# mankeyboy/ASR-FeatExt-OpenCL

Measured on NVIDIA B200. Metric: mfcc_delta_delta2_frames_per_s, higher is better.
Workload: dtype f32

## Files before the change

### asr-featext-opencl_b200/csrc/afe_fused.cuh

```cuda
#pragma once
#include <cfloat>

#include "afe_fft.cuh"
#include "afe_mel.cuh"

namespace afe {

struct Tile {
    long long pcm_off;
    long long out_row0;
    int T;
    int t0;
    int nout;
    int group;
    int tile0;
    int ntiles;
    int flags;
    int pad_;
};
constexpr int kTileNoStats = 1;
constexpr int kTileQ1All = 2;

constexpr int kMaxBanks = 64;
constexpr int kMaxWl4 = (2 * 257 + 10 * kMaxBanks + 3) / 4;
constexpr int kMagStride = 260;
__host__ __device__ constexpr int mag_row(int f) { return 8 * (f >> 3) + ((f >> 1) & 3) + 4 * (f & 1); }

struct MelConst {
    float4 wl4[kMaxWl4];
    float4 dct4[kMaxBanks][4];
    int desc[kMaxBanks];
    short wstart[8];
    int mma_unit[8][2];
    int mma_boff[8][2];
};

struct FusedArgs {
    const int16_t *pcm;
    float *out;
    const Tile *tiles;
    const float2 *window2, *tw_a, *tw_p;
    double *partials;
    int *counters;
    int cluster_norm;
    int tile_base;
    int norm_type, norm_after_dyn;
#ifdef AFE_DEVTOOLS
    int debug_skip;
#endif
    int W, S, nb, dct_len, cols, width, l1, l2, nstreams;
    int q1;
    int use_tma;
    int stats_rows_mode;
    int stats_count;
    int use_last;
    float *g_mean, *g_scale;
    int *work_counter;
    unsigned *flags;
    unsigned epoch;
    int ntiles_launch;
    float pre;
    int blk_ntiles, blk_T, blk_t_first, blk_n_out, blk_nout, blk_spec, blk_spec_q1;
    const float4 *mma_bfrag, *mma_dfrag;
    int stats_kind;
    int tc_max;
    float rden1, rden2;
};

constexpr int kRoundFrames = 32;
constexpr int kMaxFusedThreads = 256;

struct FusedSmem {
    int off_mbar, off_mags, off_part, off_warp, warp_bytes, w_pcm, w_scratch, pcm_bytes, off_dhat, off_dd, off_red,
        off_cep, total;
};

inline int align_up(int v, int a) { return (v + a - 1) / a * a; }

template <int N2>
FusedSmem fused_smem_layout(int kFusedWarps, int S, int cols, int tc_max, int nout_max, int l2, int nstreams)
{
    using C = dev::FftCfg<N2>;
    const int kWarpFrames = kRoundFrames / kFusedWarps;
    FusedSmem L;
    int o = 0;
    L.off_mbar = o; o += align_up(kFusedWarps * 8, 16);
    L.off_mags = o; o += align_up((kRoundFrames * kMagStride + 16) * 4, 16);
    L.pcm_bytes = align_up(((kWarpFrames - 1) * S + N2) * 2, 16) + 16;
    L.w_pcm = 0;
    L.warp_bytes = L.pcm_bytes;
    o = align_up(o, 128);
    L.off_warp = o; o += kFusedWarps * L.warp_bytes;
    o = align_up(o, 128);
    const int scratch = kFusedWarps * align_up(C::FPW * C::SCR * 8, 16);
    const int part = kFusedWarps * 4 * kRoundFrames * 16;
    L.w_scratch = align_up(C::FPW * C::SCR * 8, 16);
    L.off_part = o; o += scratch > part ? scratch : part;
    const int dhat = nstreams >= 2 ? align_up((nout_max + 2 * l2) * cols * 4, 16) : 0;
    const int dd = nstreams >= 3 ? align_up(nout_max * cols * 4, 16) : 0;
    L.off_dhat = L.off_mags;
    L.off_dd = L.off_dhat + dhat;
    L.off_red = L.off_dd + dd;
    const int phase3_end = L.off_red + kMaxFusedThreads * 4 * 8;
    if (phase3_end > o) o = align_up(phase3_end, 128);
    L.off_cep = o; o += align_up(tc_max * cols * 4, 16);
    L.total = o;
    return L;
}

namespace dev {

__device__ __forceinline__ uint32_t smem_u32(const void *p) { return (uint32_t)__cvta_generic_to_shared(p); }

__device__ __forceinline__ void mbar_init(uint64_t *bar, int count)
{
    asm volatile("mbarrier.init.shared::cta.b64 [%0], %1;" ::"r"(smem_u32(bar)), "r"(count));
}
__device__ __forceinline__ void mbar_expect_tx(uint64_t *bar, uint32_t bytes)
{
    asm volatile("mbarrier.arrive.expect_tx.shared::cta.b64 _, [%0], %1;" ::"r"(smem_u32(bar)), "r"(bytes) : "memory");
}
__device__ __forceinline__ void mbar_wait(uint64_t *bar, uint32_t parity)
{
    for (uint32_t spin = 0; spin < (1u << 24); spin++) {
        uint32_t done;
        asm volatile(
            "{\n\t.reg .pred p;\n\t"
            "mbarrier.try_wait.parity.shared::cta.b64 p, [%1], %2;\n\t"
            "selp.u32 %0, 1, 0, p;\n\t}"
            : "=r"(done)
            : "r"(smem_u32(bar)), "r"(parity)
            : "memory");
        if (done) return;
    }
    __trap();
}
__device__ __forceinline__ void tma_bulk_g2s(void *dst, const void *src, uint32_t bytes, uint64_t *bar)
{
    asm volatile("cp.async.bulk.shared::cluster.global.mbarrier::complete_tx::bytes [%0], [%1], %2, [%3];" ::"r"(
                     smem_u32(dst)),
                 "l"(src), "r"(bytes), "r"(smem_u32(bar))
                 : "memory");
}

__device__ __forceinline__ float4 lds128(uint32_t addr)
{
    float4 v;
    asm volatile("ld.shared.v4.f32 {%0, %1, %2, %3}, [%4];" : "=f"(v.x), "=f"(v.y), "=f"(v.z), "=f"(v.w) : "r"(addr));
    return v;
}
__device__ __forceinline__ uint32_t opaque(uint32_t v)
{
    asm volatile("" : "+r"(v));
    return v;
}

__device__ __forceinline__ void cluster_sync()
{
    asm volatile("barrier.cluster.arrive.release.aligned;\n\tbarrier.cluster.wait.acquire.aligned;" ::: "memory");
}
__device__ __forceinline__ uint32_t cluster_size()
{
    uint32_t n;
    asm volatile("mov.u32 %0, %%cluster_nctarank;" : "=r"(n));
    return n;
}
__device__ __forceinline__ double ld_peer_f64(const double *local, uint32_t rank)
{
    uint32_t peer;
    double v;
    asm volatile("mapa.shared::cluster.u32 %0, %1, %2;" : "=r"(peer) : "r"(smem_u32(local)), "r"(rank));
    asm volatile("ld.shared::cluster.f64 %0, [%1];" : "=d"(v) : "r"(peer) : "memory");
    return v;
}

__device__ __forceinline__ int clampi(int v, int lo, int hi) { return v < lo ? lo : (v > hi ? hi : v); }

}

namespace dev {

__device__ __forceinline__ float delta_num(const float *p, int stride, int L)
{
    if (L == 3) {
        float num = p[stride] - p[-stride];
        num = fmaf(2.f, p[2 * stride] - p[-2 * stride], num);
        return fmaf(3.f, p[3 * stride] - p[-3 * stride], num);
    }
    float num = 0.f;
    for (int l = 1; l <= L; l++) num = fmaf((float)l, p[l * stride] - p[-l * stride], num);
    return num;
}

template <int KIND>
__device__ __forceinline__ void write_rows(float *__restrict__ orow, const float *__restrict__ src, int r_off, int rpp, int nout,
                                           int rq, int rs, int cols, int width, int D, double &sum, double &sumsq, float &mn,
                                           float &mx)
{
    const int ostep = rpp * width, sstep = rpp * cols;
    orow += r_off * width;
    src += r_off * cols;
    for (int r = r_off; r < nout; r += rpp, orow += ostep, src += sstep) {
        const float sval = *src;
        *orow = r >= rq ? src[-D * cols] : sval;
        if (KIND >= 1 && r < rs) {
            sum += (double)sval;
            if (KIND >= 2) sumsq += (double)__fmul_rn(sval, sval);
            if (KIND >= 3) { mn = fminf(mn, sval); mx = fmaxf(mx, sval); }
        }
    }
}

template <int MODE>
__device__ __forceinline__ void phase3_l3(const int KIND, const FusedArgs &a, const Tile &tl, const float *__restrict__ s_cep,
                                          int c0f, int c1f, double *__restrict__ s_red3, int tid, int nthreads, int rs,
                                          const float *norm3 = nullptr)
{
    constexpr int R = 8;
    const int cols = a.cols, width = a.width, T = tl.T, t0 = tl.t0, nout = tl.nout;
    const int rp = nthreads / cols, g = tid / cols, c = tid - g * cols;
    if (g >= rp) return;
    const int q1 = (tl.flags & kTileQ1All) ? 2 : a.q1;
    const int rq = q1 ? (q1 == 2 ? 0 : max(0, T - 6 - t0)) : nout;
    const float rden1 = a.rden1, rden2 = a.rden2;
    double sum[3] = {0.0, 0.0, 0.0}, sumsq[3] = {0.0, 0.0, 0.0};
    float mn[3] = {FLT_MAX, FLT_MAX, FLT_MAX}, mx[3] = {-FLT_MAX, -FLT_MAX, -FLT_MAX};
    float nm[3] = {0.f, 0.f, 0.f}, ns[3] = {1.f, 1.f, 1.f};
    if (MODE == 2) {
#pragma unroll
        for (int k = 0; k < 3; k++) { nm[k] = norm3[k]; ns[k] = norm3[3 + k]; }
    }
    const bool cmn = a.norm_type == AFE_NORM_CMN;
    float *obase = a.out + (tl.out_row0 + t0) * (long long)width + c;
    for (int r0 = g * R; r0 < (MODE == 1 ? rs : nout); r0 += rp * R) {
        float x[R + 12], dh[R + 6];
#pragma unroll
        for (int i = 0; i < R + 12; i++)
            x[i] = s_cep[(clampi(t0 + r0 - 6 + i, c0f, c1f - 1) - c0f) * cols + c];
#pragma unroll
        for (int j = 0; j < R + 6; j++) {
            float num = x[j + 4] - x[j + 2];
            num = fmaf(2.f, x[j + 5] - x[j + 1], num);
            num = fmaf(3.f, x[j + 6] - x[j], num);
            dh[j] = __fmul_rn(num, rden1);
        }
        float *orow = obase + (long long)r0 * width;
#pragma unroll
        for (int r = 0; r < R; r++, orow += width) {
            const int row = r0 + r;
            if (row >= nout) break;
            float num = dh[r + 4] - dh[r + 2];
            num = fmaf(2.f, dh[r + 5] - dh[r + 1], num);
            num = fmaf(3.f, dh[r + 6] - dh[r], num);
            const float v[3] = {x[r + 6], dh[r + 3], __fmul_rn(num, rden2)};
            if (MODE == 0) {
                orow[0] = row >= rq ? x[r] : v[0];
                orow[cols] = v[1];
                orow[2 * cols] = v[2];
            } else if (MODE == 2) {
                const float w0 = row >= rq ? x[r] : v[0];
                orow[0] = cmn ? w0 - nm[0] : (w0 - nm[0]) * ns[0];
                orow[cols] = cmn ? v[1] - nm[1] : (v[1] - nm[1]) * ns[1];
                orow[2 * cols] = cmn ? v[2] - nm[2] : (v[2] - nm[2]) * ns[2];
            }
            if (MODE != 2 && KIND >= 1 && row < rs) {
#pragma unroll
                for (int k = 0; k < 3; k++) {
                    sum[k] += (double)v[k];
                    if (KIND >= 2) sumsq[k] += (double)__fmul_rn(v[k], v[k]);
                    if (KIND >= 3) { mn[k] = fminf(mn[k], v[k]); mx[k] = fmaxf(mx[k], v[k]); }
                }
            }
        }
    }
    if (MODE != 2) {
#pragma unroll
        for (int k = 0; k < 3; k++) {
            double *p = s_red3 + ((g * width) + k * cols + c) * 4;
            p[0] = sum[k]; p[1] = sumsq[k]; p[2] = (double)mn[k]; p[3] = (double)mx[k];
        }
    }
}

}

namespace dev {
__device__ __forceinline__ void mma_tf32(float (&c)[4], const uint32_t (&a)[4], uint32_t b0, uint32_t b1)
{
    asm volatile("mma.sync.aligned.m16n8k8.row.col.f32.tf32.tf32.f32 {%0, %1, %2, %3}, {%4, %5, %6, %7}, {%8, %9}, {%0, %1, %2, %3};"
                 : "+f"(c[0]), "+f"(c[1]), "+f"(c[2]), "+f"(c[3])
                 : "r"(a[0]), "r"(a[1]), "r"(a[2]), "r"(a[3]), "r"(b0), "r"(b1));
}
__device__ __forceinline__ void mma_3xtf32(float (&c)[4], const float (&av)[4], const float4 b)
{
    uint32_t ah[4], al[4];
#pragma unroll
    for (int i = 0; i < 4; i++) {
        ah[i] = __float_as_uint(av[i]) & 0xffffe000u;
        al[i] = __float_as_uint(av[i] - __uint_as_float(ah[i]));
    }
    mma_tf32(c, al, __float_as_uint(b.x), __float_as_uint(b.y));
    mma_tf32(c, ah, __float_as_uint(b.z), __float_as_uint(b.w));
    mma_tf32(c, ah, __float_as_uint(b.x), __float_as_uint(b.y));
}
}

namespace dev {
__device__ __forceinline__ Tile load_tile(const FusedArgs &a, int idx)
{
    if (a.blk_ntiles == 0) return a.tiles[idx];
    const int D = a.l1 + a.l2;
    Tile tl;
    tl.pcm_off = 0; tl.out_row0 = -(long long)a.blk_t_first; tl.T = a.blk_T; tl.group = 0; tl.tile0 = 0;
    tl.ntiles = a.blk_ntiles + a.blk_spec; tl.pad_ = 0;
    if (idx < a.blk_ntiles) {
        tl.t0 = a.blk_t_first + idx * a.blk_nout;
        tl.nout = min(a.blk_nout, a.blk_t_first + a.blk_n_out - tl.t0);
        tl.flags = 0;
    } else {
        tl.t0 = a.blk_T - D; tl.nout = D;
        tl.flags = kTileNoStats | (a.blk_spec_q1 ? kTileQ1All : 0);
    }
    return tl;
}

constexpr int kSeqTiles = 32, kSegs = 6;
__host__ __device__ inline int seg_len(int ntiles) { return ntiles <= kSeqTiles ? ntiles : (ntiles + kSegs - 1) / kSegs; }

static __device__ unsigned g_opaque_zero = 0;

__device__ __forceinline__ void sum_records(const double *__restrict__ partials, int width, int c, int t_begin, int t_end,
                                            double &s0, double &s1, double &lo, double &hi, int tstep = 1)
{
    s0 = 0.0; s1 = 0.0; lo = (double)FLT_MAX; hi = -(double)FLT_MAX;
    constexpr int U = 8;
    const size_t stride = (size_t)width * 4 * tstep;
    const double *p = partials + ((size_t)t_begin * width + c) * 4;
    const int last = t_end - 1;
    const unsigned z = *reinterpret_cast<volatile unsigned *>(&g_opaque_zero);
    for (int t = t_begin; t < t_end; t += U * tstep, p += U * stride) {
        double2 a[U], b[U];
#pragma unroll
        for (int k = 0; k < U; k++) {
            const double2 *q = reinterpret_cast<const double2 *>(t + k * tstep <= last ? p + k * stride : p);
            a[k] = q[0];
            b[k] = q[1];
        }
        unsigned all = 0;
#pragma unroll
        for (int k = 0; k < U; k++)
            all |= (unsigned)__double2hiint(a[k].x) | (unsigned)__double2hiint(a[k].y) | (unsigned)__double2hiint(b[k].x) |
                   (unsigned)__double2hiint(b[k].y);
        a[0].x = __hiloint2double(__double2hiint(a[0].x) | (int)(all & z), __double2loint(a[0].x));
#pragma unroll
        for (int k = 0; k < U; k++) {
            const bool ok = t + k * tstep <= last;
            s0 += ok ? a[k].x : 0.0; s1 += ok ? a[k].y : 0.0;
            lo = fmin(lo, ok ? b[k].x : (double)FLT_MAX); hi = fmax(hi, ok ? b[k].y : -(double)FLT_MAX);
        }
    }
}

__device__ __forceinline__ void group_total(const double *__restrict__ partials, int width, int tile0, int ntiles, int tid,
                                            int nthreads, double *s_seg, int c_of_tid, double &s0, double &s1, double &lo, double &hi)
{
    if (ntiles <= kSeqTiles) {
        if (tid < width) sum_records(partials, width, c_of_tid, tile0, tile0 + ntiles, s0, s1, lo, hi);
        return;
    }
    const int len = seg_len(ntiles);
    for (int i = tid; i < kSegs * width; i += nthreads) {
        const int seg = i / width, c = i - seg * width;
        const int b = min(ntiles, seg * len), e = min(ntiles, b + len);
        double a0, a1, l, h;
        sum_records(partials, width, c, tile0 + b, tile0 + e, a0, a1, l, h);
        double *o = s_seg + (size_t)i * 4;
        o[0] = a0; o[1] = a1; o[2] = l; o[3] = h;
    }
    __syncthreads();
    if (tid < width) {
        s0 = 0.0; s1 = 0.0; lo = (double)FLT_MAX; hi = -(double)FLT_MAX;
        for (int seg = 0; seg < kSegs; seg++) {
            const double *o = s_seg + ((size_t)seg * width + c_of_tid) * 4;
            s0 += o[0]; s1 += o[1];
            lo = fmin(lo, o[2]); hi = fmax(hi, o[3]);
        }
    }
}

__device__ __forceinline__ void normalise_tile_rows(float *__restrict__ out, const Tile &tl, int width, int norm_type,
                                                    const float *__restrict__ mean, const float *__restrict__ scale, float *s_ms)
{
    float *base = out + (tl.out_row0 + tl.t0) * (long long)width;
    const int n = tl.nout * width;
    for (int i = threadIdx.x; i < width; i += blockDim.x) {
        s_ms[i] = __ldcg(mean + (long long)tl.group * width + i);
        s_ms[width + i] = norm_type == AFE_NORM_CMN ? 1.f : __ldcg(scale + (long long)tl.group * width + i);
    }
    __syncthreads();
    const float *m = s_ms, *sc = s_ms + width;
    const bool cmn = norm_type == AFE_NORM_CMN;
    const int head = min(n, (int)(((16 - (reinterpret_cast<uintptr_t>(base) & 15)) & 15) >> 2));
    const int n4 = (n - head) >> 2, tail0 = head + 4 * n4;
    if ((int)threadIdx.x < head) {
        const int i = threadIdx.x;
        const float v = __ldcg(base + i) - m[i % width];
        base[i] = cmn ? v : v * sc[i % width];
    }
    if ((int)threadIdx.x < n - tail0) {
        const int i = tail0 + threadIdx.x, c = i % width;
        const float v = __ldcg(base + i) - m[c];
        base[i] = cmn ? v : v * sc[c];
    }
    float4 *p4 = reinterpret_cast<float4 *>(base + head);
    int c = (head + 4 * (int)threadIdx.x) % width;
    const int cstep = (4 * (int)blockDim.x) % width;
    constexpr int U = 4;
    const int bd = blockDim.x;
    for (int j = threadIdx.x; j < n4; j += U * bd) {
        float4 v[U];
#pragma unroll
        for (int k = 0; k < U; k++)
            if (j + k * bd < n4) v[k] = __ldcg(p4 + j + k * bd);
#pragma unroll
        for (int k = 0; k < U; k++) {
            if (j + k * bd < n4) {
                int c1 = c + 1; if (c1 >= width) c1 -= width;
                int c2 = c1 + 1; if (c2 >= width) c2 -= width;
                int c3 = c2 + 1; if (c3 >= width) c3 -= width;
                float4 w = v[k];
                w.x -= m[c]; w.y -= m[c1]; w.z -= m[c2]; w.w -= m[c3];
                if (!cmn) { w.x *= sc[c]; w.y *= sc[c1]; w.z *= sc[c2]; w.w *= sc[c3]; }
                p4[j + k * bd] = w;
            }
            c += cstep; if (c >= width) c -= width;
        }
    }
}

__device__ __forceinline__ void normalise_role(const FusedArgs &a, const Tile tl, float *s_ms)
{
    if (threadIdx.x == 0) {
        unsigned v = 0;
        for (unsigned spin = 0; spin < (1u << 26); spin++) {
            asm volatile("ld.acquire.gpu.global.u32 %0, [%1];" : "=r"(v) : "l"(a.flags + tl.group) : "memory");
            if (v == a.epoch) break;
            __nanosleep(128);
        }
        if (v != a.epoch) __trap();
    }
    __syncthreads();
    normalise_tile_rows(a.out, tl, a.width, a.norm_type, a.g_mean, a.g_scale, s_ms);
}
}

template <int N2, int NZ, int kFusedWarps, int KF, bool PRE, bool MMA = false>
__global__ void __launch_bounds__(32 * kFusedWarps, 2)
k_fused_mfcc(const FusedArgs a, const FusedSmem L, const __grid_constant__ MelConst mc)
{
    constexpr bool FAST = false;
    using C = dev::FftCfg<N2>;
    constexpr int kFusedThreads = 32 * kFusedWarps, kWarpFrames = kRoundFrames / kFusedWarps;
    constexpr int R = C::R, FPW = C::FPW, SCR = C::SCR;
    static_assert(kWarpFrames % FPW == 0, "a warp's frames must fill whole FFT calls");
    extern __shared__ __align__(128) unsigned char smem[];
    float *s_mags = reinterpret_cast<float *>(smem + L.off_mags);
    float *s_cep = reinterpret_cast<float *>(smem + L.off_cep);

    const int tid = threadIdx.x, lane = tid & 31;
    const int warp = __shfl_sync(0xffffffffu, tid >> 5, 0);
    const int lf = lane % R, fw = lane / R;
    unsigned char *wbase = smem + L.off_warp + warp * L.warp_bytes;
    uint64_t *w_mbar = reinterpret_cast<uint64_t *>(smem + L.off_mbar) + warp;
    unsigned char *w_pcm = wbase + L.w_pcm;
    float2 *w_scratch = reinterpret_cast<float2 *>(smem + L.off_part + warp * L.w_scratch);

    int tile_local = blockIdx.x;
    if (a.work_counter) {
        __shared__ int s_role;
        if (tid == 0) {
            const int t = atomicAdd(a.work_counter, 1);
            if (t == (int)gridDim.x - 1) *a.work_counter = 0;
            s_role = t;
        }
        __syncthreads();
        tile_local = s_role;
        if (tile_local >= a.ntiles_launch) {
            const int n_norm = (int)gridDim.x - a.ntiles_launch;
            for (int j = tile_local - a.ntiles_launch; j < a.ntiles_launch; j += n_norm) {
                dev::normalise_role(a, dev::load_tile(a, a.tile_base + j), reinterpret_cast<float *>(smem));
                __syncthreads();
            }
            return;
        }
    }
    const int tile_idx = a.tile_base + tile_local;
    const Tile tl = dev::load_tile(a, tile_idx);
    const int q1 = (tl.flags & kTileQ1All) ? 2 : a.q1;
    const int D = a.l1 + a.l2, cols = a.cols;
    const int c0f = max(0, tl.t0 - D), c1f = min(tl.T, tl.t0 + tl.nout + D);
    const int ncomp = c1f - c0f;
    const int nrounds = (ncomp + kRoundFrames - 1) / kRoundFrames;
    const int16_t *wpcm = a.pcm + tl.pcm_off + (long long)(c0f + warp * kWarpFrames) * a.S;
    auto warp_frames = [&](int r) { return min(kWarpFrames, ncomp - r * kRoundFrames - warp * kWarpFrames); };
    auto issue_tma = [&](int r) {
        const int nf = warp_frames(r);
        if (nf <= 0) return;
        const uint32_t bytes = (uint32_t)((((nf - 1) * a.S + a.W) * 2 + 15) & ~15);
        asm volatile("fence.proxy.async.shared::cta;" ::: "memory");
        dev::mbar_expect_tx(w_mbar, bytes);
        dev::tma_bulk_g2s(w_pcm, wpcm + (long long)r * kRoundFrames * a.S, bytes, w_mbar);
    };
    if (a.use_tma && lane == 0) {
        dev::mbar_init(w_mbar, 1);
        asm volatile("fence.mbarrier_init.release.cluster;" ::: "memory");
        issue_tma(0);
    }
    dev::LaneConsts<N2, NZ> lc;
    dev::load_lane_consts<N2, NZ>(lc, a.window2, a.tw_a, a.tw_p, lf);
    for (int i = tid; i < (kRoundFrames * kMagStride + 16) / 4; i += kFusedThreads)
        reinterpret_cast<float4 *>(s_mags)[i] = make_float4(0.f, 0.f, 0.f, 0.f);
    __syncthreads();

    const uint32_t mrow_s = dev::opaque(dev::smem_u32(s_mags) + mag_row(lane) * kMagStride * 4);
    uint32_t parity = 0;
    for (int r = 0; r < nrounds; r++) {
        const int f0 = r * kRoundFrames;
        const int nfr = min(kRoundFrames, ncomp - f0);
        const int nfw = warp_frames(r);
        if (nfw > 0) {
            if (a.use_tma) {
                dev::mbar_wait(w_mbar, parity);
                parity ^= 1;
            } else {
                const int16_t *src = wpcm + (long long)f0 * a.S;
                const int n = (nfw - 1) * a.S + a.W;
                int16_t *dst = reinterpret_cast<int16_t *>(w_pcm);
                if ((reinterpret_cast<uintptr_t>(src) & 3) == 0) {
                    const uint32_t *s32 = reinterpret_cast<const uint32_t *>(src);
                    uint32_t *d32 = reinterpret_cast<uint32_t *>(dst);
                    for (int i = lane; i < n / 2; i += 32) d32[i] = __ldg(s32 + i);
                    if ((n & 1) && lane == 0) dst[n - 1] = src[n - 1];
                } else
                    for (int i = lane; i < n; i += 32) dst[i] = src[i];
                __syncwarp();
            }
#pragma unroll
            for (int it = 0; it < kWarpFrames / FPW; it++) {
                if (it * FPW >= nfw) break;
#ifdef AFE_DEVTOOLS
                if (a.debug_skip & 1) break;
#endif
                const int fl = it * FPW + fw;
                const int fr = warp * kWarpFrames + fl;
                const uint32_t *words = reinterpret_cast<const uint32_t *>(w_pcm) + ((fl * a.S) >> 1);
                dev::fft_frame_mag<N2, NZ, true, false, PRE>(words, lc, w_scratch + fw * SCR, s_mags + mag_row(fr) * kMagStride, lf, a.pre);
            }
            if (a.use_tma && lane == 0 && r + 1 < nrounds) issue_tma(r + 1);
        }
        __syncthreads();

        if constexpr (MMA) {
            const int g = lane >> 2, t = lane & 3;
#pragma unroll 1
            for (int ui = 0; ui < 2; ui++) {
                const int ud = mc.mma_unit[warp][ui];
                if (ud < 0) break;
                const int m = ud & 1, j = (ud >> 4) & 15, s0 = (ud >> 8) & 255, ns = (ud >> 16) & 255;
                const float4 *bf = a.mma_bfrag + (size_t)mc.mma_boff[warp][ui] * 32 + lane;
                const int row = 16 * m + (g >> 1) + 4 * (g & 1);
                const float *r0 = s_mags + row * kMagStride + 8 * s0 + t, *r1 = r0 + 8 * kMagStride;
                float e[4] = {0.f, 0.f, 0.f, 0.f};
#pragma unroll 2
                for (int s = 0; s < ns; s++, r0 += 8, r1 += 8, bf += 32) {
                    const float4 b = __ldg(bf);
                    const float av[4] = {r0[0], r1[0], r0[4], r1[4]};
                    dev::mma_3xtf32(e, av, b);
                }
                const float2 l01 = dev::mel_log2<FAST>(make_float2(e[0], e[1])), l23 = dev::mel_log2<FAST>(make_float2(e[2], e[3]));
                if (a.dct_len > 0) {
                    const float lv[4] = {l01.x, l23.x, l01.y, l23.y};
#pragma unroll
                    for (int ct = 0; ct < 2; ct++) {
                        float dd[4] = {0.f, 0.f, 0.f, 0.f};
                        dev::mma_3xtf32(dd, lv, __ldg(a.mma_dfrag + (j * 2 + ct) * 32 + lane));
                        float *part = reinterpret_cast<float *>(smem + L.off_part + (2 * m + ct) * L.w_scratch) + (j * 16 + g) * 8 + 2 * t;
                        *reinterpret_cast<float2 *>(part) = make_float2(dd[0], dd[1]);
                        *reinterpret_cast<float2 *>(part + 64) = make_float2(dd[2], dd[3]);
                    }
                } else {
                    const int fa = 16 * m + g, fb = fa + 8, b0 = 8 * j + 2 * t;
                    if (fa < nfr) {
                        if (b0 < a.nb) s_cep[(f0 + fa) * cols + b0] = l01.x;
                        if (b0 + 1 < a.nb) s_cep[(f0 + fa) * cols + b0 + 1] = l01.y;
                    }
                    if (fb < nfr) {
                        if (b0 < a.nb) s_cep[(f0 + fb) * cols + b0] = l23.x;
                        if (b0 + 1 < a.nb) s_cep[(f0 + fb) * cols + b0 + 1] = l23.y;
                    }
                }
            }
        } else
        #ifdef AFE_DEVTOOLS
        if (lane < nfr && !(a.debug_skip & 2)) {
#else
        if (lane < nfr) {
#endif
            float es[KF];
            int woff = mc.wstart[warp];
            int dsc[KF];
            float4 mf0[KF], mf1[KF];
#pragma unroll
            for (int k = 0; k < KF; k++) {
                const int b = warp + k * kFusedWarps;
                dsc[k] = b < a.nb ? mc.desc[b] : 0;
                const uint32_t maddr = mrow_s + ((dsc[k] & 0xffff) << 4);
                mf0[k] = dev::lds128(maddr);
                mf1[k] = dev::lds128(maddr + 16);
            }
#pragma unroll
            for (int k = 0; k < KF; k++) {
                float2 acc0 = make_float2(0.f, 0.f), acc1 = acc0;
                int n8 = dsc[k] >> 16;
                if (n8 > 0) {
                    uint32_t maddr = mrow_s + ((dsc[k] & 0xffff) << 4);
                    float4 m0 = mf0[k], m1 = mf1[k];
                    for (;;) {
                        const float4 w0 = mc.wl4[woff], w1 = mc.wl4[woff + 1];
                        acc0 = __ffma2_rn(make_float2(m0.x, m0.y), make_float2(w0.x, w0.y), acc0);
                        acc1 = __ffma2_rn(make_float2(m0.z, m0.w), make_float2(w0.z, w0.w), acc1);
                        acc0 = __ffma2_rn(make_float2(m1.x, m1.y), make_float2(w1.x, w1.y), acc0);
                        acc1 = __ffma2_rn(make_float2(m1.z, m1.w), make_float2(w1.z, w1.w), acc1);
                        woff += 2;
                        if (--n8 == 0) break;
                        maddr += 32;
                        m0 = dev::lds128(maddr);
                        m1 = dev::lds128(maddr + 16);
                    }
                }
                const float2 t = __fadd2_rn(acc0, acc1);
                es[k] = t.x + t.y;
            }
#pragma unroll
            for (int k = 0; k + 1 < KF; k += 2) {
                const float2 e2 = dev::mel_log2<FAST>(make_float2(es[k], es[k + 1]));
                es[k] = e2.x; es[k + 1] = e2.y;
            }
            if (KF & 1) es[KF - 1] = dev::mel_log<FAST>(es[KF - 1]);
            if (a.dct_len > 0) {
                float2 cep[8];
#pragma unroll
                for (int c = 0; c < 8; c++) cep[c] = make_float2(0.f, 0.f);
#pragma unroll
                for (int k = 0; k < KF; k++) {
                    const int b = warp + k * kFusedWarps;
                    const float2 e2 = make_float2(es[k], es[k]);
#pragma unroll
                    for (int c4 = 0; c4 < 4; c4++) {
                        const float4 d4 = mc.dct4[b][c4];
                        cep[2 * c4 + 0] = __ffma2_rn(e2, make_float2(d4.x, d4.y), cep[2 * c4 + 0]);
                        cep[2 * c4 + 1] = __ffma2_rn(e2, make_float2(d4.z, d4.w), cep[2 * c4 + 1]);
                    }
                }
#pragma unroll
                for (int c4 = 0; c4 < 4; c4++)
                    reinterpret_cast<float4 *>(smem + L.off_part + c4 * L.w_scratch)[warp * kRoundFrames + lane] =
                        make_float4(cep[2 * c4].x, cep[2 * c4].y, cep[2 * c4 + 1].x, cep[2 * c4 + 1].y);
            } else {
#pragma unroll
                for (int k = 0; k < KF; k++)
                    if (warp + k * kFusedWarps < a.nb) s_cep[(f0 + lane) * cols + warp + k * kFusedWarps] = es[k];
            }
        }
        __syncthreads();
        if (MMA) {
            if (a.dct_len > 0 && warp < 4) {
                const int nt = (a.nb + 7) >> 3, fr = 16 * (warp >> 1) + (lane >> 1), c0 = 8 * (warp & 1) + 4 * (lane & 1);
                const float4 *part = reinterpret_cast<const float4 *>(w_scratch) + (lane >> 1) * 2 + (lane & 1);
                float4 tsum = part[0];
                for (int j = 1; j < nt; j++) {
                    const float4 u = part[j * 32];
                    tsum.x += u.x; tsum.y += u.y; tsum.z += u.z; tsum.w += u.w;
                }
                if (fr < nfr) {
                    float *crow = s_cep + (f0 + fr) * cols + c0;
                    if (c0 + 0 < a.dct_len) crow[0] = tsum.x;
                    if (c0 + 1 < a.dct_len) crow[1] = tsum.y;
                    if (c0 + 2 < a.dct_len) crow[2] = tsum.z;
                    if (c0 + 3 < a.dct_len) crow[3] = tsum.w;
                }
                __syncwarp();
            }
        } else if (a.dct_len > 0 && warp < 4) {
            if (lane < nfr) {
                const float4 *part = reinterpret_cast<const float4 *>(w_scratch);
                float4 t = part[lane];
#pragma unroll
                for (int w2 = 1; w2 < kFusedWarps; w2++) {
                    const float4 u = part[w2 * kRoundFrames + lane];
                    t.x += u.x; t.y += u.y; t.z += u.z; t.w += u.w;
                }
                float *crow = s_cep + (f0 + lane) * cols + 4 * warp;
                if (4 * warp + 0 < a.dct_len) crow[0] = t.x;
                if (4 * warp + 1 < a.dct_len) crow[1] = t.y;
                if (4 * warp + 2 < a.dct_len) crow[2] = t.z;
                if (4 * warp + 3 < a.dct_len) crow[3] = t.w;
            }
            __syncwarp();
        }
    }
    __syncthreads();

    float *s_dhat = reinterpret_cast<float *>(smem + L.off_dhat);
    float *s_dd = reinterpret_cast<float *>(smem + L.off_dd);
    double *s_red = reinterpret_cast<double *>(smem + L.off_red);
    const int T = tl.T, t0 = tl.t0, nout = tl.nout, l1 = a.l1, l2 = a.l2;
#ifdef AFE_DEVTOOLS
    if (a.debug_skip & 4) return;
#endif
    const int width = a.width;
    const int rpp = kFusedThreads / width;
    const bool active = tid < rpp * width;
    const int r_off = tid / width, col = tid - r_off * width;
    const int strm = col / cols, c = col - strm * cols;
    const int n_stats = a.stats_rows_mode == 1 ? T - D : a.stats_rows_mode == 2 ? T : a.stats_rows_mode == 3 ? a.stats_count : 0;
    const float *src = strm == 0 ? s_cep + (t0 - c0f) * cols + c : strm == 1 ? s_dhat + l2 * cols + c : s_dd + c;
    const int rq = (q1 && strm == 0) ? (q1 == 2 ? 0 : max(0, T - D - t0)) : nout;
    const int rs = (tl.flags & kTileNoStats) ? 0 : a.stats_rows_mode == 3 ? nout : min(nout, max(0, n_stats - t0));
    const bool fast3 = a.nstreams == 3 && l1 == 3 && l2 == 3;
    if (fast3 && a.use_last) {
        const int cc = tid % cols;
        const float *gm = a.g_mean + (long long)tl.group * width, *gs = a.g_scale + (long long)tl.group * width;
        const float norm3[6] = {gm[cc], gm[cols + cc], gm[2 * cols + cc], gs[cc], gs[cols + cc], gs[2 * cols + cc]};
        dev::phase3_l3<2>(0, a, tl, s_cep, c0f, c1f, nullptr, tid, kFusedThreads, rs, norm3);
    } else if (fast3 && a.cluster_norm) {
        double *s_red3 = reinterpret_cast<double *>(smem + L.off_mags);
        double *s_rec = reinterpret_cast<double *>(smem + L.off_mags + 25 * 1024);
        float *s_mean = reinterpret_cast<float *>(smem + L.off_mags + 30 * 1024), *s_scale = s_mean + width;
        dev::phase3_l3<1>(a.stats_kind, a, tl, s_cep, c0f, c1f, s_red3, tid, kFusedThreads, rs);
        __syncthreads();
        if (tid < width) {
            const int rp = kFusedThreads / cols;
            double s0 = 0.0, s1 = 0.0, lo = (double)FLT_MAX, hi = -(double)FLT_MAX;
            for (int g = 0; g < rp; g++) {
                const double *p = s_red3 + (g * width + tid) * 4;
                s0 += p[0]; s1 += p[1];
                lo = fmin(lo, p[2]); hi = fmax(hi, p[3]);
            }
            double *rec = s_rec + tid * 4;
            rec[0] = s0; rec[1] = s1; rec[2] = lo; rec[3] = hi;
        }
        dev::cluster_sync();
        if (tid < width) {
            const double *rec = s_rec + (a.norm_after_dyn ? tid : tid % cols) * 4;
            const uint32_t ncta = dev::cluster_size();
            double s0 = 0.0, s1 = 0.0, lo = (double)FLT_MAX, hi = -(double)FLT_MAX;
            for (uint32_t t = 0; t < ncta; t++) {
                s0 += dev::ld_peer_f64(rec, t); s1 += dev::ld_peer_f64(rec + 1, t);
                lo = fmin(lo, dev::ld_peer_f64(rec + 2, t)); hi = fmax(hi, dev::ld_peer_f64(rec + 3, t));
            }
            const double n = (double)n_stats;
            float m = (float)(s0 / n), sc = 1.f;
            if (a.norm_type == AFE_NORM_CVN) sc = (float)sqrt((n - 1.0) / (s1 - s0 * (s0 / n)));
            else if (a.norm_type == AFE_NORM_MINMAX) sc = 1.f / fmaxf(fabsf((float)lo - m), fabsf((float)hi - m));
            if (!a.norm_after_dyn && tid >= cols) m = 0.f;
            s_mean[tid] = m; s_scale[tid] = sc;
            if (a.g_mean && tile_idx == tl.tile0) {
                a.g_mean[(long long)tl.group * width + tid] = m;
                a.g_scale[(long long)tl.group * width + tid] = sc;
            }
        }
        __syncthreads();
        {
            const int cc = tid % cols;
            const float norm3[6] = {s_mean[cc], s_mean[cols + cc], s_mean[2 * cols + cc],
                                    s_scale[cc], s_scale[cols + cc], s_scale[2 * cols + cc]};
            dev::phase3_l3<2>(0, a, tl, s_cep, c0f, c1f, s_red3, tid, kFusedThreads, rs, norm3);
        }
        dev::cluster_sync();
    } else if (fast3) {
        double *s_red3 = reinterpret_cast<double *>(smem + L.off_mags);
        dev::phase3_l3<0>(a.stats_kind, a, tl, s_cep, c0f, c1f, s_red3, tid, kFusedThreads, rs);
        if (a.partials) {
            __syncthreads();
            if (tid < width) {
                const int rp = kFusedThreads / cols;
                double s0 = 0.0, s1 = 0.0, lo = (double)FLT_MAX, hi = -(double)FLT_MAX;
                for (int g = 0; g < rp; g++) {
                    const double *p = s_red3 + (g * width + tid) * 4;
                    s0 += p[0]; s1 += p[1];
                    lo = fmin(lo, p[2]); hi = fmax(hi, p[3]);
                }
                double *dst = a.partials + ((long long)tile_idx * width + tid) * 4;
                dst[0] = s0; dst[1] = s1; dst[2] = lo; dst[3] = hi;
            }
        }
    } else {
        if (a.nstreams >= 2) {
            const int rp = kFusedThreads / cols, rl = tid / cols, c = tid - rl * cols;
            const int nd = nout + 2 * l2;
            if (rl < rp) {
                for (int i = rl; i < nd; i += rp) {
                    const int u = t0 - l2 + i;
                    float num;
                    if (u - l1 >= 0 && u + l1 <= T - 1)
                        num = dev::delta_num(s_cep + (u - c0f) * cols + c, cols, l1);
                    else {
                        num = 0.f;
                        for (int l = 1; l <= l1; l++) {
                            const float hi = s_cep[(dev::clampi(u + l, 0, T - 1) - c0f) * cols + c];
                            const float lo = s_cep[(dev::clampi(u - l, 0, T - 1) - c0f) * cols + c];
                            num = fmaf((float)l, hi - lo, num);
                        }
                    }
                    s_dhat[i * cols + c] = num * a.rden1;
                }
            }
            __syncthreads();
            if (a.nstreams >= 3) {
                if (rl < rp)
                    for (int r = rl; r < nout; r += rp)
                        s_dd[r * cols + c] = dev::delta_num(s_dhat + (r + l2) * cols + c, cols, l2) * a.rden2;
                __syncthreads();
            }
        }

        double sum = 0.0, sumsq = 0.0;
        float mn = FLT_MAX, mx = -FLT_MAX;
        if (active) {
            float *orow = a.out + (tl.out_row0 + t0) * (long long)width + col;
            switch (a.stats_kind) {
            case 0: dev::write_rows<0>(orow, src, r_off, rpp, nout, rq, rs, cols, width, D, sum, sumsq, mn, mx); break;
            case 1: dev::write_rows<1>(orow, src, r_off, rpp, nout, rq, rs, cols, width, D, sum, sumsq, mn, mx); break;
            case 2: dev::write_rows<2>(orow, src, r_off, rpp, nout, rq, rs, cols, width, D, sum, sumsq, mn, mx); break;
            default: dev::write_rows<3>(orow, src, r_off, rpp, nout, rq, rs, cols, width, D, sum, sumsq, mn, mx); break;
            }
        }
        if (a.partials) {
            s_red[tid * 4 + 0] = sum;
            s_red[tid * 4 + 1] = sumsq;
            s_red[tid * 4 + 2] = (double)mn;
            s_red[tid * 4 + 3] = (double)mx;
            __syncthreads();
            if (tid < width) {
                double s0 = 0.0, s1 = 0.0, lo = (double)FLT_MAX, hi = -(double)FLT_MAX;
                for (int g = 0; g < rpp; g++) {
                    const double *p = s_red + (g * width + tid) * 4;
                    s0 += p[0]; s1 += p[1];
                    lo = fmin(lo, p[2]); hi = fmax(hi, p[3]);
                }
                double *dst = a.partials + ((long long)tile_idx * width + tid) * 4;
                dst[0] = s0; dst[1] = s1; dst[2] = lo; dst[3] = hi;
            }
        }
        if (a.use_last) {
            __syncthreads();
            dev::normalise_tile_rows(a.out, tl, width, a.norm_type, a.g_mean, a.g_scale, reinterpret_cast<float *>(smem + L.off_dhat));
        }
    }

    if (a.counters) {
        __shared__ int s_last;
        float *s_mean = reinterpret_cast<float *>(smem + L.off_dhat), *s_scale = s_mean + width;
        __threadfence();
        __syncthreads();
        if (tid == 0) {
            const int ticket = atomicAdd(a.counters + tl.group, 1);
            s_last = ticket == tl.ntiles - 1;
            if (s_last) a.counters[tl.group] = 0;
        }
        __syncthreads();
        if (s_last) {
            __threadfence();
            double s0, s1, lo, hi;
            {
                double *s_seg = reinterpret_cast<double *>(smem + L.off_mags + 1024);
                const int src_col = a.norm_after_dyn ? tid : tid % cols;
                dev::group_total(a.partials, width, tl.tile0, tl.ntiles, tid, kFusedThreads, s_seg, tid < width ? src_col : 0, s0, s1, lo, hi);
            }
            if (tid < width) {
                const double n = (double)n_stats;
                float m = (float)(s0 / n), sc = 1.f;
                if (a.norm_type == AFE_NORM_CVN) sc = (float)sqrt((n - 1.0) / (s1 - s0 * (s0 / n)));
                else if (a.norm_type == AFE_NORM_MINMAX) sc = 1.f / fmaxf(fabsf((float)lo - m), fabsf((float)hi - m));
                if (!a.norm_after_dyn && tid >= cols) m = 0.f;
                s_mean[tid] = m; s_scale[tid] = sc;
                if (a.g_mean) {
                    a.g_mean[(long long)tl.group * width + tid] = m;
                    a.g_scale[(long long)tl.group * width + tid] = sc;
                }
            }
            if (a.work_counter) {
                __threadfence();
                __syncthreads();
                if (tid == 0) asm volatile("st.release.gpu.global.u32 [%0], %1;" ::"l"(a.flags + tl.group), "r"(a.epoch) : "memory");
                return;
            }
            __syncthreads();
            if (active) {
                const Tile tf = dev::load_tile(a, tl.tile0), tz = dev::load_tile(a, tl.tile0 + tl.ntiles - 1);
                const int rb = tf.t0, re = tz.t0 + tz.nout;
                float *o = a.out + (tl.out_row0 + rb) * (long long)width + col;
                const float m = s_mean[col], sc = a.norm_type == AFE_NORM_CMN ? 1.f : s_scale[col];
                const bool cmn = a.norm_type == AFE_NORM_CMN;
                const int step = rpp * width;
                o += r_off * width;
                int r = rb + r_off;
                constexpr int U = 8;
                for (; r + (U - 1) * rpp < re; r += U * rpp, o += U * step) {
                    float v[U];
#pragma unroll
                    for (int k = 0; k < U; k++) v[k] = __ldcg(o + k * step);
#pragma unroll
                    for (int k = 0; k < U; k++) o[k * step] = cmn ? v[k] - m : (v[k] - m) * sc;
                }
                for (; r < re; r += rpp, o += step) *o = cmn ? __ldcg(o) - m : (__ldcg(o) - m) * sc;
            }
        }
    }
}

}
```

Before: 1.595 billion.

## Stage fused MFCC delta rows in shared memory and store normalized output vectorized

```diff
diff --git a/asr-featext-opencl_b200/csrc/afe_fused.cuh b/asr-featext-opencl_b200/csrc/afe_fused.cuh
--- a/asr-featext-opencl_b200/csrc/afe_fused.cuh
+++ b/asr-featext-opencl_b200/csrc/afe_fused.cuh
@@ -72,7 +72,7 @@
 
 struct FusedSmem {
     int off_mbar, off_mags, off_part, off_warp, warp_bytes, w_pcm, w_scratch, pcm_bytes, off_dhat, off_dd, off_red,
-        off_cep, total;
+        off_rows, off_cep, off_red3, total;
 };
 
 inline int align_up(int v, int a) { return (v + a - 1) / a * a; }
@@ -96,14 +96,19 @@
     const int part = kFusedWarps * 4 * kRoundFrames * 16;
     L.w_scratch = align_up(C::FPW * C::SCR * 8, 16);
     L.off_part = o; o += scratch > part ? scratch : part;
+    const int width = nstreams * cols;
     const int dhat = nstreams >= 2 ? align_up((nout_max + 2 * l2) * cols * 4, 16) : 0;
     const int dd = nstreams >= 3 ? align_up(nout_max * cols * 4, 16) : 0;
     L.off_dhat = L.off_mags;
     L.off_dd = L.off_dhat + dhat;
     L.off_red = L.off_dd + dd;
-    const int phase3_end = L.off_red + kMaxFusedThreads * 4 * 8;
+    L.off_rows = L.off_mags;
+    const int generic_end = L.off_red + kMaxFusedThreads * 4 * 8, rows_end = L.off_rows + (nout_max * width + 3) * 4;
+    const int phase3_end = generic_end > rows_end ? generic_end : rows_end;
     if (phase3_end > o) o = align_up(phase3_end, 128);
-    L.off_cep = o; o += align_up(tc_max * cols * 4, 16);
+    const int rec3 = (32 * kFusedWarps / cols) * width * 32 + width * 32 + 2 * width * 4;
+    const int cep = tc_max * cols * 4;
+    L.off_cep = o; L.off_red3 = o; o += align_up(cep > rec3 ? cep : rec3, 16);
     L.total = o;
     return L;
 }
@@ -211,28 +216,32 @@
     }
 }
 
-template <int MODE>
+struct Stats3 {
+    double sum[3], sumsq[3];
+    float mn[3], mx[3];
+    __device__ __forceinline__ void store(double *s_red3, int g, int width, int cols, int c) const
+    {
+#pragma unroll
+        for (int k = 0; k < 3; k++) {
+            double *p = s_red3 + ((g * width) + k * cols + c) * 4;
+            p[0] = sum[k]; p[1] = sumsq[k]; p[2] = (double)mn[k]; p[3] = (double)mx[k];
+        }
+    }
+};
+
 __device__ __forceinline__ void phase3_l3(const int KIND, const FusedArgs &a, const Tile &tl, const float *__restrict__ s_cep,
-                                          int c0f, int c1f, double *__restrict__ s_red3, int tid, int nthreads, int rs,
-                                          const float *norm3 = nullptr)
+                                          int c0f, int c1f, float *__restrict__ rows, Stats3 &st, int tid, int nthreads, int rs)
 {
     constexpr int R = 8;
     const int cols = a.cols, width = a.width, T = tl.T, t0 = tl.t0, nout = tl.nout;
     const int rp = nthreads / cols, g = tid / cols, c = tid - g * cols;
-    if (g >= rp) return;
     const int q1 = (tl.flags & kTileQ1All) ? 2 : a.q1;
     const int rq = q1 ? (q1 == 2 ? 0 : max(0, T - 6 - t0)) : nout;
     const float rden1 = a.rden1, rden2 = a.rden2;
-    double sum[3] = {0.0, 0.0, 0.0}, sumsq[3] = {0.0, 0.0, 0.0};
-    float mn[3] = {FLT_MAX, FLT_MAX, FLT_MAX}, mx[3] = {-FLT_MAX, -FLT_MAX, -FLT_MAX};
-    float nm[3] = {0.f, 0.f, 0.f}, ns[3] = {1.f, 1.f, 1.f};
-    if (MODE == 2) {
-#pragma unroll
-        for (int k = 0; k < 3; k++) { nm[k] = norm3[k]; ns[k] = norm3[3 + k]; }
-    }
-    const bool cmn = a.norm_type == AFE_NORM_CMN;
-    float *obase = a.out + (tl.out_row0 + t0) * (long long)width + c;
-    for (int r0 = g * R; r0 < (MODE == 1 ? rs : nout); r0 += rp * R) {
+#pragma unroll
+    for (int k = 0; k < 3; k++) { st.sum[k] = 0.0; st.sumsq[k] = 0.0; st.mn[k] = FLT_MAX; st.mx[k] = -FLT_MAX; }
+    if (g >= rp) return;
+    for (int r0 = g * R; r0 < nout; r0 += rp * R) {
         float x[R + 12], dh[R + 6];
 #pragma unroll
         for (int i = 0; i < R + 12; i++)
@@ -244,7 +253,7 @@
             num = fmaf(3.f, x[j + 6] - x[j], num);
             dh[j] = __fmul_rn(num, rden1);
         }
-        float *orow = obase + (long long)r0 * width;
+        float *orow = rows + (long long)r0 * width + c;
 #pragma unroll
         for (int r = 0; r < R; r++, orow += width) {
             const int row = r0 + r;
@@ -253,32 +262,52 @@
             num = fmaf(2.f, dh[r + 5] - dh[r + 1], num);
             num = fmaf(3.f, dh[r + 6] - dh[r], num);
             const float v[3] = {x[r + 6], dh[r + 3], __fmul_rn(num, rden2)};
-            if (MODE == 0) {
-                orow[0] = row >= rq ? x[r] : v[0];
-                orow[cols] = v[1];
-                orow[2 * cols] = v[2];
-            } else if (MODE == 2) {
-                const float w0 = row >= rq ? x[r] : v[0];
-                orow[0] = cmn ? w0 - nm[0] : (w0 - nm[0]) * ns[0];
-                orow[cols] = cmn ? v[1] - nm[1] : (v[1] - nm[1]) * ns[1];
-                orow[2 * cols] = cmn ? v[2] - nm[2] : (v[2] - nm[2]) * ns[2];
-            }
-            if (MODE != 2 && KIND >= 1 && row < rs) {
+            orow[0] = row >= rq ? x[r] : v[0];
+            orow[cols] = v[1];
+            orow[2 * cols] = v[2];
+            if (KIND >= 1 && row < rs) {
 #pragma unroll
                 for (int k = 0; k < 3; k++) {
-                    sum[k] += (double)v[k];
-                    if (KIND >= 2) sumsq[k] += (double)__fmul_rn(v[k], v[k]);
-                    if (KIND >= 3) { mn[k] = fminf(mn[k], v[k]); mx[k] = fmaxf(mx[k], v[k]); }
-                }
-            }
-        }
-    }
-    if (MODE != 2) {
-#pragma unroll
-        for (int k = 0; k < 3; k++) {
-            double *p = s_red3 + ((g * width) + k * cols + c) * 4;
-            p[0] = sum[k]; p[1] = sumsq[k]; p[2] = (double)mn[k]; p[3] = (double)mx[k];
-        }
+                    st.sum[k] += (double)v[k];
+                    if (KIND >= 2) st.sumsq[k] += (double)__fmul_rn(v[k], v[k]);
+                    if (KIND >= 3) { st.mn[k] = fminf(st.mn[k], v[k]); st.mx[k] = fmaxf(st.mx[k], v[k]); }
+                }
+            }
+        }
+    }
+}
+
+__device__ __forceinline__ void store_rows(float *__restrict__ out, const float *__restrict__ s_tile, int n, int width,
+                                           const float *mean, const float *scale, bool cmn, int tid, int nthreads)
+{
+    const int e = (int)((reinterpret_cast<uintptr_t>(out) >> 2) & 3);
+    const int head = min(n, (4 - e) & 3);
+    const int n4 = (n - head) >> 2, tail0 = head + 4 * n4;
+    auto one = [&](int i) {
+        const int c = i % width;
+        const float v = s_tile[i] - mean[c];
+        out[i] = cmn ? v : v * scale[c];
+    };
+    if (tid < head) one(tid);
+    if (tid < n - tail0) one(tail0 + tid);
+    const int period = (width & 3) == 0 ? width >> 2 : (width & 1) ? width : width >> 1;
+    const int nv = nthreads / period * period;
+    if (tid >= nv) return;
+    int cq[4];
+    cq[0] = (head + 4 * tid) % width;
+#pragma unroll
+    for (int q = 1; q < 4; q++) cq[q] = cq[q - 1] + 1 == width ? 0 : cq[q - 1] + 1;
+    const float2 m01 = make_float2(-mean[cq[0]], -mean[cq[1]]), m23 = make_float2(-mean[cq[2]], -mean[cq[3]]);
+    float2 s01 = make_float2(1.f, 1.f), s23 = s01;
+    if (!cmn) { s01 = make_float2(scale[cq[0]], scale[cq[1]]); s23 = make_float2(scale[cq[2]], scale[cq[3]]); }
+    const float4 *src = reinterpret_cast<const float4 *>(s_tile + head);
+    float4 *dst = reinterpret_cast<float4 *>(out + head);
+#pragma unroll 4
+    for (int j = tid; j < n4; j += nv) {
+        const float4 v = src[j];
+        float2 lo = __fadd2_rn(make_float2(v.x, v.y), m01), hi = __fadd2_rn(make_float2(v.z, v.w), m23);
+        if (!cmn) { lo = __fmul2_rn(lo, s01); hi = __fmul2_rn(hi, s23); }
+        dst[j] = make_float4(lo.x, lo.y, hi.x, hi.y);
     }
 }
 
@@ -728,72 +757,72 @@
     const int rq = (q1 && strm == 0) ? (q1 == 2 ? 0 : max(0, T - D - t0)) : nout;
     const int rs = (tl.flags & kTileNoStats) ? 0 : a.stats_rows_mode == 3 ? nout : min(nout, max(0, n_stats - t0));
     const bool fast3 = a.nstreams == 3 && l1 == 3 && l2 == 3;
-    if (fast3 && a.use_last) {
-        const int cc = tid % cols;
-        const float *gm = a.g_mean + (long long)tl.group * width, *gs = a.g_scale + (long long)tl.group * width;
-        const float norm3[6] = {gm[cc], gm[cols + cc], gm[2 * cols + cc], gs[cc], gs[cols + cc], gs[2 * cols + cc]};
-        dev::phase3_l3<2>(0, a, tl, s_cep, c0f, c1f, nullptr, tid, kFusedThreads, rs, norm3);
-    } else if (fast3 && a.cluster_norm) {
-        double *s_red3 = reinterpret_cast<double *>(smem + L.off_mags);
-        double *s_rec = reinterpret_cast<double *>(smem + L.off_mags + 25 * 1024);
-        float *s_mean = reinterpret_cast<float *>(smem + L.off_mags + 30 * 1024), *s_scale = s_mean + width;
-        dev::phase3_l3<1>(a.stats_kind, a, tl, s_cep, c0f, c1f, s_red3, tid, kFusedThreads, rs);
-        __syncthreads();
-        if (tid < width) {
-            const int rp = kFusedThreads / cols;
-            double s0 = 0.0, s1 = 0.0, lo = (double)FLT_MAX, hi = -(double)FLT_MAX;
-            for (int g = 0; g < rp; g++) {
-                const double *p = s_red3 + (g * width + tid) * 4;
-                s0 += p[0]; s1 += p[1];
-                lo = fmin(lo, p[2]); hi = fmax(hi, p[3]);
-            }
-            double *rec = s_rec + tid * 4;
-            rec[0] = s0; rec[1] = s1; rec[2] = lo; rec[3] = hi;
-        }
-        dev::cluster_sync();
-        if (tid < width) {
-            const double *rec = s_rec + (a.norm_after_dyn ? tid : tid % cols) * 4;
-            const uint32_t ncta = dev::cluster_size();
-            double s0 = 0.0, s1 = 0.0, lo = (double)FLT_MAX, hi = -(double)FLT_MAX;
-            for (uint32_t t = 0; t < ncta; t++) {
-                s0 += dev::ld_peer_f64(rec, t); s1 += dev::ld_peer_f64(rec + 1, t);
-                lo = fmin(lo, dev::ld_peer_f64(rec + 2, t)); hi = fmax(hi, dev::ld_peer_f64(rec + 3, t));
-            }
-            const double n = (double)n_stats;
-            float m = (float)(s0 / n), sc = 1.f;
-            if (a.norm_type == AFE_NORM_CVN) sc = (float)sqrt((n - 1.0) / (s1 - s0 * (s0 / n)));
-            else if (a.norm_type == AFE_NORM_MINMAX) sc = 1.f / fmaxf(fabsf((float)lo - m), fabsf((float)hi - m));
-            if (!a.norm_after_dyn && tid >= cols) m = 0.f;
-            s_mean[tid] = m; s_scale[tid] = sc;
-            if (a.g_mean && tile_idx == tl.tile0) {
-                a.g_mean[(long long)tl.group * width + tid] = m;
-                a.g_scale[(long long)tl.group * width + tid] = sc;
-            }
-        }
-        __syncthreads();
-        {
-            const int cc = tid % cols;
-            const float norm3[6] = {s_mean[cc], s_mean[cols + cc], s_mean[2 * cols + cc],
-                                    s_scale[cc], s_scale[cols + cc], s_scale[2 * cols + cc]};
-            dev::phase3_l3<2>(0, a, tl, s_cep, c0f, c1f, s_red3, tid, kFusedThreads, rs, norm3);
-        }
-        dev::cluster_sync();
-    } else if (fast3) {
-        double *s_red3 = reinterpret_cast<double *>(smem + L.off_mags);
-        dev::phase3_l3<0>(a.stats_kind, a, tl, s_cep, c0f, c1f, s_red3, tid, kFusedThreads, rs);
-        if (a.partials) {
+    if (fast3) {
+        float *gtile = a.out + (tl.out_row0 + t0) * (long long)width;
+        const int rp = kFusedThreads / cols, g = tid / cols;
+        dev::Stats3 st;
+        if (!a.cluster_norm && !a.use_last) {
+            dev::phase3_l3(a.stats_kind, a, tl, s_cep, c0f, c1f, gtile, st, tid, kFusedThreads, rs);
+            if (a.partials) {
+                double *s_red3 = reinterpret_cast<double *>(smem + L.off_mags);
+                if (g < rp) st.store(s_red3, g, width, cols, tid - g * cols);
+                __syncthreads();
+                if (tid < width) {
+                    double s0 = 0.0, s1 = 0.0, lo = (double)FLT_MAX, hi = -(double)FLT_MAX;
+                    for (int gg = 0; gg < rp; gg++) {
+                        const double *p = s_red3 + (gg * width + tid) * 4;
+                        s0 += p[0]; s1 += p[1];
+                        lo = fmin(lo, p[2]); hi = fmax(hi, p[3]);
+                    }
+                    double *dst = a.partials + ((long long)tile_idx * width + tid) * 4;
+                    dst[0] = s0; dst[1] = s1; dst[2] = lo; dst[3] = hi;
+                }
+            }
+        } else {
+            float *s_rows = reinterpret_cast<float *>(smem + L.off_rows) + ((reinterpret_cast<uintptr_t>(gtile) >> 2) & 3);
+            double *s_red3 = reinterpret_cast<double *>(smem + L.off_red3), *s_rec = s_red3 + rp * width * 4;
+            float *s_mean = reinterpret_cast<float *>(s_rec + width * 4), *s_scale = s_mean + width;
+            dev::phase3_l3(a.use_last ? 0 : a.stats_kind, a, tl, s_cep, c0f, c1f, s_rows, st, tid, kFusedThreads, rs);
             __syncthreads();
-            if (tid < width) {
-                const int rp = kFusedThreads / cols;
-                double s0 = 0.0, s1 = 0.0, lo = (double)FLT_MAX, hi = -(double)FLT_MAX;
-                for (int g = 0; g < rp; g++) {
-                    const double *p = s_red3 + (g * width + tid) * 4;
-                    s0 += p[0]; s1 += p[1];
-                    lo = fmin(lo, p[2]); hi = fmax(hi, p[3]);
-                }
-                double *dst = a.partials + ((long long)tile_idx * width + tid) * 4;
-                dst[0] = s0; dst[1] = s1; dst[2] = lo; dst[3] = hi;
-            }
+            const float *mean = a.g_mean + (long long)tl.group * width, *scale = a.g_scale + (long long)tl.group * width;
+            if (a.cluster_norm) {
+                if (g < rp) st.store(s_red3, g, width, cols, tid - g * cols);
+                __syncthreads();
+                if (tid < width) {
+                    double s0 = 0.0, s1 = 0.0, lo = (double)FLT_MAX, hi = -(double)FLT_MAX;
+                    for (int gg = 0; gg < rp; gg++) {
+                        const double *p = s_red3 + (gg * width + tid) * 4;
+                        s0 += p[0]; s1 += p[1];
+                        lo = fmin(lo, p[2]); hi = fmax(hi, p[3]);
+                    }
+                    double *rec = s_rec + tid * 4;
+                    rec[0] = s0; rec[1] = s1; rec[2] = lo; rec[3] = hi;
+                }
+                dev::cluster_sync();
+                if (tid < width) {
+                    const double *rec = s_rec + (a.norm_after_dyn ? tid : tid % cols) * 4;
+                    const uint32_t ncta = dev::cluster_size();
+                    double s0 = 0.0, s1 = 0.0, lo = (double)FLT_MAX, hi = -(double)FLT_MAX;
+                    for (uint32_t t = 0; t < ncta; t++) {
+                        s0 += dev::ld_peer_f64(rec, t); s1 += dev::ld_peer_f64(rec + 1, t);
+                        lo = fmin(lo, dev::ld_peer_f64(rec + 2, t)); hi = fmax(hi, dev::ld_peer_f64(rec + 3, t));
+                    }
+                    const double n = (double)n_stats;
+                    float m = (float)(s0 / n), sc = 1.f;
+                    if (a.norm_type == AFE_NORM_CVN) sc = (float)sqrt((n - 1.0) / (s1 - s0 * (s0 / n)));
+                    else if (a.norm_type == AFE_NORM_MINMAX) sc = 1.f / fmaxf(fabsf((float)lo - m), fabsf((float)hi - m));
+                    if (!a.norm_after_dyn && tid >= cols) m = 0.f;
+                    s_mean[tid] = m; s_scale[tid] = sc;
+                    if (a.g_mean && tile_idx == tl.tile0) {
+                        a.g_mean[(long long)tl.group * width + tid] = m;
+                        a.g_scale[(long long)tl.group * width + tid] = sc;
+                    }
+                }
+                __syncthreads();
+                mean = s_mean; scale = s_scale;
+            }
+            dev::store_rows(gtile, s_rows, nout * width, width, mean, scale, a.norm_type == AFE_NORM_CMN, tid, kFusedThreads);
+            if (a.cluster_norm) dev::cluster_sync();
         }
     } else {
         if (a.nstreams >= 2) {
```

Result: faster. 1.629 billion, median of 6 (+2.1%).
